# keiserlab/amyloid-yolo-paper

Hardware: AMD Instinct MI355X
Metric: tiles/sec (1024x1024 RGB) inference (higher is better)
Workload: dtype bf16; 1 GPU; configs[1]: Darknet-53+FPN YOLOv3, batch=64 synthetic 1024x1024 tiles/GPU, C=3, seeded random weights, decode + merge-NMS on (conf 0.5, nms 0.4); global_batch=64, tile=1024, parallelism=replicas x1 (tiles sharded by image, no collective)

## Files before the change

### amyloid_yolo_paper_amd/_lib.py

```python
import ctypes as C
import os

HERE = os.path.dirname(os.path.abspath(__file__))
LIB_PATH = os.path.join(HERE, "libamyloid_yolo_hip.so")
ABI_VERSION = 2


class ConvDesc(C.Structure):
    _fields_ = [(n, C.c_int32) for n in (
        "batch", "cin", "cout", "hin", "win", "hout", "wout", "ksize", "stride", "leaky", "out_f32", "cout_pad")]


class PlanOp(C.Structure):
    _fields_ = [("kind", C.c_int32), ("src", C.c_int32), ("src2", C.c_int32), ("res", C.c_int32), ("dst", C.c_int32),
                ("conv", ConvDesc), ("c1", C.c_int32), ("c2", C.c_int32), ("up1", C.c_int32), ("leaky2", C.c_int32),
                ("num_anchors", C.c_int32), ("num_classes", C.c_int32), ("grid", C.c_int32), ("row_offset", C.c_int32),
                ("anchors_wh", C.c_float * 12),
                ("w", C.c_void_p), ("scale", C.c_void_p), ("shift", C.c_void_p),
                ("w2", C.c_void_p), ("scale2", C.c_void_p), ("shift2", C.c_void_p)]


class AugParams(C.Structure):
    _fields_ = [("src_offset", C.c_int64), ("h", C.c_int32), ("w", C.c_int32), ("inv", C.c_float * 6), ("flip", C.c_int32),
                ("sharpen_alpha", C.c_float), ("drop_threshold", C.c_uint32), ("drop_seed", C.c_uint32),
# ... 43 lines not shown
    "ay_bn_train_bwd_f32": (_I, [_P, _P, _P, _P, _P, _P, _I, _P, _P, _P, _I, _I, _I, _P]),
    "ay_bias_grad_f32": (_I, [_P, _P, _I, _I, _I, _P]),
    "ay_bias_grad_f32_acc": (_I, [_P, _P, _I, _I, _I, _I, _P]),
    "ay_conv_dgrad_f32": (_I, [C.POINTER(ConvDesc), _P, _P, _P, _I, _P]),
    "ay_conv_wgrad_f32": (_I, [C.POINTER(ConvDesc), _P, _P, _P, _P]),
    "ay_add_f32": (_I, [_P, _P, _P, _SZ, _P]),
    "ay_accumulate_f32": (_I, [_P, _P, _SZ, _P]),
    "ay_copy_channels_f32": (_I, [_P, _P, _I, _I, _I, _I, _I, _I, _I, _P]),
    "ay_slice_accumulate_f32": (_I, [_P, _P, _I, _I, _I, _I, _I, _I, _I, _P]),
    "ay_yolo_loss_workspace_bytes": (_SZ, [_I, _I, _I, _I]),
    "ay_yolo_loss_fwd_bwd": (_I, [_P, _P, _I, _I, _I, _I, _I, _I, C.POINTER(C.c_float), _F, _F, _P, _P, _P, _SZ, _P]),
    "ay_conv1x1_cat_fwd_bf16": (_I, [C.POINTER(ConvDesc), _P, _I, _P, _P, _P, _P, _P, _P]),
    "ay_resblock_supported": (_I, [_I]),
    "ay_plan_create": (_I, [C.POINTER(PlanOp), _I, C.POINTER(C.c_size_t), _I, _I, _I, _I, C.POINTER(C.c_void_p)]),
    "ay_plan_destroy": (None, [_P]),
    "ay_plan_workspace_bytes": (_SZ, [_P]),
    "ay_plan_value_offset": (_SZ, [_P, _I]),
    "ay_plan_forward": (_I, [_P, _P, _P, _P, _P]),
    "ay_plan_forward_timed": (_I, [_P, _P, _P, _P, C.POINTER(C.c_float), _P]),
    "ay_plan_profile_begin": (_I, [_P, C.POINTER(C.c_ubyte)]),
    "ay_plan_profile_begin_every": (_I, [_P, C.POINTER(C.c_ubyte), _I]),
    "ay_plan_profile_end": (_I, [_P, C.POINTER(C.c_float), C.POINTER(C.c_int)]),
    "ay_resblock_fwd_bf16": (_I, [_P, _P, _P, _P, _I, _P, _P, _P, _I, _P, _I, _I, _I, _I, _P]),
    "ay_match_detections": (_I, [_P, _P, _I, _I, _P, _I, _F, _P, _P, _P]),
    "ay_ingest_tiles_u8": (_I, [_P, _I, _I, _I, _I, _F, _P, _P]),
    "ay_ingest_region_tiles_u8": (_I, [_P, _I, _I, _SZ, _I, _I, _I, _I, _I, _P, _P]),
    "ay_ingest_region_tiles_step_u8": (_I, [_P, _I, _I, _SZ, _I, _I, _I, _I, _I, _I, _P, _P]),
    "ay_ingest_region_tiles_list_u8": (_I, [_P, _I, _I, _SZ, _I, _I, _P, _I, _I, _P, _P]),
    "ay_augment_ingest_u8": (_I, [_P, _SZ, _P, _I, _I, _P, _P]),
    "ay_augment_ingest_window_u8": (_I, [_P, _SZ, _P, _I, _I, _P, _P]),
# ... 99 lines not shown
```

### amyloid_yolo_paper_amd/csrc/ay_conv3x3_m16.hip

```cpp
#include <type_traits>

#include "ay_conv_common.h"

namespace ay {

#ifdef AY_PHASE_CLOCK
__device__ unsigned long long g_phase_ticks_m16[10];
#define AY_CLK(...) __VA_ARGS__
#else
#define AY_CLK(...)
#endif

template <bool HAS_RES, typename DT = Bf16>
__global__ void __launch_bounds__(512, 2) conv3x3_m16_ring_kernel(ConvArgs a, int n_items) {
    DT::enter();
    typedef typename DT::vec8 vec8;
    constexpr int BN = 128, TH = 16, TW = 32;
    constexpr int IN_W = TW + 2, IN_PIX = (TH + 2) * IN_W;
    constexpr int IN_PIXP = (IN_PIX + 15) / 16 * 16;
    constexpr int PX_PIECES = (2 * IN_PIXP + 63) / 64;
    constexpr int PIX_SLAB = PX_PIECES * 1024;
    constexpr int W_PIECES = 9 * 2 * BN * 16 / 1024;
    constexpr int W_SLAB = W_PIECES * 1024;
    constexpr int W_BASE = PIX_SLAB;
// ... 5 lines not shown
    constexpr int SS_BASE = DUMMY_BASE + 1024;
    constexpr int MBOX_BASE = SS_BASE + 4 * 2048;
    constexpr int LDS_BYTES = MBOX_BASE + 64;
    static_assert(LDS_BYTES <= 160 * 1024, "LDS ring");
    constexpr int MT = 4, NT = 8;

    __shared__ __attribute__((aligned(16))) uint8_t lds[LDS_BYTES];
    __builtin_amdgcn_s_setprio(2);

    const int tid = threadIdx.x;
    const int lane = tid & 63;
    const int wave = __builtin_amdgcn_readfirstlane(tid >> 6);
    const int wm = wave & 1, wn = wave >> 1;
    const int r = lane & 15, g = lane >> 4, h = g & 1, hi = g >> 1;

    const ItemRange rg(n_items);
    const int last = rg.last;
    int item = rg.first_item();
    const ItemDealer dealer(rg, a.deal, lds + MBOX_BASE, 3);
    if (item >= last) {
        dealer.leave();
        return;
    }
    dealer.post_first();
    int seq_l = 0, seq_c = 0;

    const size_t in_plane = (size_t)a.hin * a.win * 32;
    const int CP = a.cout_pad;
    const size_t w_stage_stride = (size_t)9 * 2 * CP * 16;
    const int tiles_per_img = a.tiles_x * a.tiles_y;
    const unsigned lds_base = lds_addr_of(lds);
    const int nstages = a.cin / 16;

    constexpr unsigned OOB = 0x80000000u;
    unsigned px_off[PWP];
    const uint8_t* ld_src = nullptr;
    int ld_cg = 0;
    int ld_item = item, ld_s = 0, ld_par = 0;
    bool ld_done = false;
    auto setup_loader = [&](int it) __attribute__((always_inline)) {
        ld_cg = it % a.n_cgroups;
        const int pt = it / a.n_cgroups;
        const int b = pt / tiles_per_img;
        const int y0 = ((pt / a.tiles_x) % a.tiles_y) * TH, x0 = (pt % a.tiles_x) * TW;
        ld_src = a.src + (size_t)b * (a.cin / 16) * in_plane;
#pragma unroll
        for (int i = 0; i < PWP; ++i) {
            const int q = i * 8 + wave;
            const int u = q * 64 + lane;
            const int hh = u / IN_PIXP, P = u % IN_PIXP;
            const int iy = y0 - 1 + P / IN_W, ix = x0 - 1 + P % IN_W;
            const bool in = q < PX_PIECES && hh < 2 && P < IN_PIX && iy >= 0 && iy < a.hin && ix >= 0 && ix < a.win;
            px_off[i] = in ? (unsigned)((iy * a.win + ix) * 32 + hh * 16) : OOB;
        }
    };
// ... 39 lines not shown
    const int was = W_BASE + ((16 + h) * BN + wm * 64 + r) * 16 + hi * BUF_BYTES;

    setup_loader(item);
#pragma unroll
    for (int i = 0; i < PW; ++i) issue_piece(i, 0);
    advance_loader();
    asm volatile("s_waitcnt vmcnt(0)" ::: "memory");
    __builtin_amdgcn_s_barrier();
    asm volatile("" ::: "memory");

    int par = 0;
    AY_CLK(const bool clk = (a.dbg & 8) && wave == 0; unsigned long long tk_stage = 0, tk_epi = 0, tk_items = 0, tk_wait = 0, tk_wait0 = 0, tk_str = 0, tk0 = 0, tkw = 0;
           const unsigned long long tk_begin = wall_clock64();)
    while (true) {
        AY_CLK(if (clk) tk0 = wall_clock64();)
        const int cg = item % a.n_cgroups;
        const int pt = item / a.n_cgroups;
        const int b = pt / tiles_per_img;
        const int y0 = ((pt / a.tiles_x) % a.tiles_y) * TH, x0 = (pt % a.tiles_x) * TW;
        const int next_item = dealer.id_at(seq_c + 1);
        const bool has_next = next_item < last;

        f32x4 acc[MT][NT];
#pragma unroll
        for (int m = 0; m < MT; ++m)
#pragma unroll
            for (int n = 0; n < NT; ++n) acc[m][n] = f32x4{0.f, 0.f, 0.f, 0.f};

        typedef __attribute__((address_space(3))) const f32x4 lds_f4;
        lds_f4* sl4 = (lds_f4*)(__attribute__((address_space(3))) const float*)(lds + SS_BASE + par * 2048);
        const float slope = a.leaky ? 0.1f : 1.0f;
        const size_t out_plane_px = (size_t)a.hout * a.wout;
// ... 233 lines not shown
```

### amyloid_yolo_paper_amd/csrc/ay_conv_bf16.hip

```cpp
#include <stdlib.h>

#include <atomic>
#include <mutex>

#include "ay_conv_common.h"

namespace ay {

template <int KS, int STRIDE, int BN, int WM, int WN, int TH, int TW, int NK, bool OUT_F32, bool HAS_RES, typename DT = Bf16, bool DECODE = false>
__global__ void __launch_bounds__(256, 2) conv_bf16_kernel(ConvArgs a, DecodeArgs dd) {
    DT::enter();
    typedef typename DT::vec8 vec8;
    constexpr int PAD = (KS - 1) / 2;
    constexpr int KK2 = KS * KS;
    constexpr int NPIX = TH * TW;
    constexpr int NT = NPIX / (WN * 32);
    constexpr int MT = BN / (WM * 32);
    constexpr int IN_H = (TH - 1) * STRIDE + KS;
    constexpr int IN_W = (TW - 1) * STRIDE + KS;
    constexpr int IN_PIX = IN_H * IN_W;
    constexpr int PIX_SLAB = 2 * IN_PIX * 16;
    constexpr int W_SLAB = KK2 * 2 * BN * 16;
    constexpr int W_BASE = NK * PIX_SLAB;
    constexpr int LDS_BYTES = NK * (PIX_SLAB + W_SLAB);
// ... 1 lines not shown
    constexpr int NPXU = (PXU_TOTAL + 255) / 256;
    constexpr int WU_TOTAL = NK * KK2 * 2 * BN;
    constexpr int NWU = (WU_TOTAL + 255) / 256;
    static_assert(WM * WN == 4 && NT >= 1 && MT >= 1, "4 waves");
    static_assert(NT * WN * 32 == NPIX && MT * WM * 32 == BN, "tile split");
    static_assert(LDS_BYTES <= 80 * 1024, "two workgroups per CU");

    __shared__ __attribute__((aligned(16))) uint8_t lds[LDS_BYTES];

    const int tid = threadIdx.x;
    const int lane = tid & 63;
    const int wave = tid >> 6;
    const int wm = wave % WM, wn = wave / WM;
    const int c = lane & 31, hh = lane >> 5;

    const int bid = blockIdx.x;
    const int cg = bid % a.n_cgroups;
    const int pt = bid / a.n_cgroups;
    const int tile_x = pt % a.tiles_x;
    const int tile_y = (pt / a.tiles_x) % a.tiles_y;
    const int b = pt / (a.tiles_x * a.tiles_y);
    const int y0 = tile_y * TH, x0 = tile_x * TW;

    const size_t in_plane = (size_t)a.hin * a.win * 32;
    const uint8_t* src_img = a.src + (size_t)b * (a.cin / 16) * in_plane;
    const int CP = a.cout_pad;
    const uint8_t* wbase = a.w + (size_t)cg * BN * 16;
    const size_t w_stage_stride = (size_t)NK * KK2 * 2 * CP * 16;

    int px_off[NPXU];
#pragma unroll
// ... 155 lines not shown
    static_assert(WM * WN == 8 && NT >= 1 && MT >= 1, "8 waves");
    static_assert(NT * WN * 32 == NPIX && MT * WM * 32 == BN, "tile split");
    static_assert((KK2 * 2 * BN * 16) % 1024 == 0, "filter slab is whole DMA pieces");
    static_assert(LDS_BYTES <= 160 * 1024, "LDS ring");
    static_assert(NBUF == 2 || NBUF == 3, "ring depth");

    __shared__ __attribute__((aligned(16))) uint8_t lds[LDS_BYTES];
    __builtin_amdgcn_s_setprio(2);

    const int tid = threadIdx.x;
    const int lane = tid & 63;
    const int wave = __builtin_amdgcn_readfirstlane(tid >> 6);
    const int wm = wave % WM, wn = wave / WM;
    const int c = lane & 31, hh = lane >> 5;

    const ItemRange rg(n_items);
    const int last = rg.last;
    int item = rg.first_item();
    const ItemDealer dealer(rg, a.deal, lds + MBOX_BASE, (a.cin / (16 * NK)) >= 2 ? 3 : 5);
    if (item >= last) {
        dealer.leave();
        return;
    }
    dealer.post_first();
    int seq_l = 0, seq_c = 0;

    const size_t in_plane = (size_t)a.hin * a.win * 32;
    const int CP = a.cout_pad;
    const size_t w_stage_stride = (size_t)NK * KK2 * 2 * CP * 16;
    const int tiles_per_img = a.tiles_x * a.tiles_y;
    const unsigned lds_base = lds_addr_of(lds);
// ... 18 lines not shown
    for (int i = 0; i < PWW; ++i) {
        const int qq = i * 8 + wave;
        const int u = qq * 64 + lane;
        const int r = u % BN, th = u / BN;
        unsigned off = OOB;
        if (qq < NK * W_PIECES) {
            if constexpr (PAIR)
                off = (unsigned)((th * CP + r % (BN / 2)) * 16) + (unsigned)(r / (BN / 2)) * a.w_class_stride;
            else
                off = (unsigned)((th * CP + r) * 16);
        } else if (qq < NK * W_PIECES + SSP && lane < BN / 4) {
            off = (unsigned)(((lane * 4) % BNR) * 4);
        }
        w_off[i] = off;
    }
    auto setup_loader = [&](int it) __attribute__((always_inline)) {
        int cg = it % a.n_cgroups;
        const int pt = it / a.n_cgroups;
        const int b = pt / tiles_per_img;
        const int y0 = ((pt / a.tiles_x) % a.tiles_y) * TH, x0 = (pt % a.tiles_x) * TW;
        ld_src = a.src + (size_t)b * src_planes * in_plane;
        if constexpr (CAT) ld_src1 = a.src1 + (size_t)b * (a.c1 / 16) * in_plane1;
        const uint8_t* wbase = a.w;
        if constexpr (PAIR) {
            wbase += (size_t)((cg & 1) * 2) * a.w_class_stride;
            cg >>= 1;
        } else if constexpr (UP2) {
            wbase += (size_t)(cg & 3) * a.w_class_stride;
            cg >>= 2;
        }
        ld_w = wbase + (size_t)cg * BNR * 16;
// ... 96 lines not shown
            asm volatile("s_waitcnt vmcnt(0)" ::: "memory");
        }
    } else {
        asm volatile("s_waitcnt vmcnt(0)" ::: "memory");
    }
    __builtin_amdgcn_s_barrier();
    asm volatile("" ::: "memory");

    int cur = 0;
    int par = 0;
    const bool clk = AY_DBGBIT(a, 8) && wave == 0;
    unsigned long long tk_stage = 0, tk_epi = 0, tk_items = 0, tk0 = 0, tk_begin = 0, tk_s0 = 0, tk_w0 = 0, tk_w = 0, tk_nw = 0, tkw = 0;
    if (clk) tk_begin = wall_clock64();
    while (true) {
        if (clk) tk0 = wall_clock64();
        int cg = item % a.n_cgroups;
        const int cls = PAIR ? (cg & 1) * 2 : UP2 ? (cg & 3) : 0;
        if constexpr (PAIR)
            cg >>= 1;
        else if constexpr (UP2)
            cg >>= 2;
        const int pt = item / a.n_cgroups;
        const int b = pt / tiles_per_img;
        const int y0 = ((pt / a.tiles_x) % a.tiles_y) * TH, x0 = (pt % a.tiles_x) * TW;
        const int next_item = dealer.id_at(seq_c + 1);
        const bool has_next = next_item < last;

        f32x16 acc[MT][NT];
#pragma unroll
        for (int m = 0; m < MT; ++m)
#pragma unroll
            for (int n = 0; n < NT; ++n)
#pragma unroll
                for (int r = 0; r < 16; ++r) acc[m][n][r] = 0.f;
        ResRegs<MT, NT> rr;

        for (int s = 0; s < nstages; ++s) {
// ... 186 lines not shown
    a.cout_pad = d->cout_pad;
    a.hin = d->hin;
    a.win = d->win;
    a.hout = d->hout;
    a.wout = d->wout;
    a.tiles_x = (d->wout + TW - 1) / TW;
    a.tiles_y = (d->hout + TH - 1) / TH;
    a.n_cgroups = d->cout_pad / BN;
    a.leaky = d->leaky;
    a.dbg = 0;
    a.src1 = nullptr;
    a.c1 = 0;
    a.deal = nullptr;
    a.canvas_gx = 0;
    a.w_class_stride = 0;
}

int conv_dbg() {
    static const int dbg = getenv("AY_DBG") ? atoi(getenv("AY_DBG")) : 0;
    return dbg;
}

unsigned persistent_grid(long long n_items, int wgs_per_cu) {
    if (n_items <= 0 || n_items > 0x7fffffffLL) return 0;
    const long long per_xcd = (n_items + 7) / 8;
    const long long cu_slots = (long long)wgs_per_cu * (conv_num_cus() / 8);
    return (unsigned)(8 * (per_xcd < cu_slots ? per_xcd : cu_slots));
}

static long long plan_tiles(ConvArgs& a, const ay_conv_desc* d, int th, int tw, bool canvas_ok) {
    int ctx = 0, cty = 0;
// ... 251 lines not shown
```

### amyloid_yolo_paper_amd/csrc/ay_conv_common.h

```cpp
#pragma once
#include "ay_common.h"

#ifdef AY_PHASE_CLOCK
#define AY_DBGBIT(a, bit) ((a).dbg & (bit))
#else
#define AY_DBGBIT(a, bit) 0
#endif

namespace ay {

struct ConvArgs {
    const uint8_t* src;
    const uint8_t* w;
    const float* scale;
    const float* shift;
    const uint8_t* residual;
    uint8_t* out;
    int batch, cin, cout_pad, hin, win, hout, wout;
    int tiles_x, tiles_y, n_cgroups;
    int leaky;
    int dbg;
    const uint8_t* src1;
    int c1;
    unsigned* deal;
    int canvas_gx;
    unsigned w_class_stride;
};

struct DecodeArgs {
    float* pred;
    int n_total;
    int row_offset;
    int A, K;
    float stride;
    float aw[6], ah[6];
};

struct ItemRange {
    int xcd, slot, slots, first, last;
    __device__ __forceinline__ explicit ItemRange(int n_items) {
        xcd = blockIdx.x & 7, slot = blockIdx.x >> 3, slots = gridDim.x >> 3;
        const int per_xcd = (n_items + 7) >> 3;
        first = xcd * per_xcd;
        last = min(first + per_xcd, n_items);
    }
    __device__ __forceinline__ int first_item() const { return first + slot; }
};

struct ItemDealer {
    typedef volatile __attribute__((address_space(3))) int lds_vint;
    const ItemRange& rg;
    unsigned* deal;
    lds_vint* mbox;
    int D;
    __device__ __forceinline__ ItemDealer(const ItemRange& rg, unsigned* deal, void* mbox_lds, int D)
        : rg(rg), deal(deal), mbox((lds_vint*)(__attribute__((address_space(3))) int*)mbox_lds), D(D) {}
    __device__ __forceinline__ void leave() const {
        if (deal != nullptr && threadIdx.x == 0) {
            const unsigned d = atomicAdd(deal + 8, 1u);
            if (d == gridDim.x - 1) {
#pragma unroll
// ... 274 lines not shown
                } else {
#pragma unroll
                    for (int j = 0; j < 4; ++j) {
                        const int ch = ch0 + j;
                        const int an = ch / dd.K, k = ch - an * dd.K;
                        if (ch < dd.A * dd.K) rows[(size_t)an * G * G * dd.K + k] = res[j];
                    }
                }
            }
        }
    }
}

int conv_num_cus();
int conv_dbg();
unsigned* next_deal_set(hipStream_t st);
void fill_args(ConvArgs& a, const ay_conv_desc* d, const void* src, const void* w, const float* scale, const float* shift,
               const void* residual, void* out, int TH, int TW, int BN);
unsigned persistent_grid(long long n_items, int wgs_per_cu = 1);

inline int launch_ring(void (*kernel)(ConvArgs, int), ConvArgs a, long long n_items, bool dynamic, hipStream_t st, const char* what,
                       const char* kernel_name) {
    const unsigned grid = persistent_grid(n_items);
    if (!grid) {
        set_error("%s grid out of range (%lld)", what, n_items);
        return AY_ERR_ARG;
    }
    a.deal = dynamic ? next_deal_set(st) : nullptr;
    hipLaunchKernelGGL(kernel, dim3(grid), dim3(512), 0, st, a, (int)n_items);
    AY_CHECK_LAUNCH(kernel_name);
// ... 5 lines not shown
```

### amyloid_yolo_paper_amd/csrc/ay_plan.hip

```cpp
#include <hip/hip_runtime.h>

#include <algorithm>
#include <cstring>
#include <mutex>
#include <vector>

#include "ay_common.h"

struct ay_plan {
    std::vector<ay_plan_op> ops;
    std::vector<size_t> bytes, offset;
    std::vector<int> def_op, last_use;
    size_t arena = 0;
    int img_dim = 0, n_total = 0;
    int dtype = AY_DT_BF16;
    std::vector<int> fused;
    mutable bool profiling = false;
    mutable int prof_every = 1, prof_seen = 0;
    mutable std::vector<std::vector<hipEvent_t>> prof_events;
    std::vector<unsigned char> prof_sel;
};

namespace {

constexpr size_t ALIGN = 256;

bool uses_src2(int kind) { return kind == AY_OP_CONV1X1_CAT || kind == AY_OP_CONCAT_UPSAMPLE; }

void op_reads(const ay_plan_op& o, int (&r)[3]) {
    r[0] = (o.kind == AY_OP_STEM_S2_FUSED || o.kind == AY_OP_STEM) ? AY_PLAN_NONE : o.src;
    r[1] = uses_src2(o.kind) ? o.src2 : AY_PLAN_NONE;
// ... 1 lines not shown
}

struct Entries {
    decltype(&ay_head_decode_fwd_bf16) head_decode;
    decltype(&ay_stem_s2_fused_fwd) stem_s2_fused;
    decltype(&ay_stem_conv_fwd) stem;
    decltype(&ay_conv_fwd_bf16) conv;
    decltype(&ay_resblock_fwd_bf16) resblock;
    decltype(&ay_conv1x1_cat_fwd_bf16) conv1x1_cat;
};
constexpr Entries ENTRIES_BF16 = {ay_head_decode_fwd_bf16, ay_stem_s2_fused_fwd, ay_stem_conv_fwd,
                                  ay_conv_fwd_bf16,        ay_resblock_fwd_bf16, ay_conv1x1_cat_fwd_bf16};
constexpr Entries ENTRIES_F16 = {ay_head_decode_fwd_f16, ay_stem_s2_fused_fwd_f16, ay_stem_conv_fwd_f16,
                                 ay_conv_fwd_f16,        ay_resblock_fwd_f16,      ay_conv1x1_cat_fwd_f16};

int issue(const ay_plan* p, size_t idx, const float* x, uint8_t* ws, float* out, ay_stream_t st) {
    const ay_plan_op& o = p->ops[idx];
    const Entries& fn = p->dtype == AY_DT_F16 ? ENTRIES_F16 : ENTRIES_BF16;
    auto at = [&](int v) -> void* { return v >= 0 ? ws + p->offset[v] : nullptr; };
    const ay_conv_desc& d = o.conv;
    if (p->fused[idx] < 0) return AY_OK;
    if (p->fused[idx] > 0) {
        const ay_plan_op& y = p->ops[p->fused[idx]];
        return fn.head_decode(&d, at(o.src), o.w, o.scale, o.shift, y.num_anchors, y.num_classes, p->img_dim, y.anchors_wh, out,
                              p->n_total, y.row_offset, st);
    }
    switch (o.kind) {
        case AY_OP_STEM_S2_FUSED:
            return fn.stem_s2_fused(x, o.w, o.scale, o.shift, d.leaky, o.w2, o.scale2, o.shift2, o.leaky2, at(o.dst), d.batch, p->img_dim,
                                    p->img_dim, st);
        case AY_OP_STEM:
// ... 3 lines not shown
        case AY_OP_RESBLOCK:
            return fn.resblock(at(o.src), o.w, o.scale, o.shift, d.leaky, o.w2, o.scale2, o.shift2, o.leaky2, at(o.dst), d.batch, d.cin,
                               d.hout, d.wout, st);
        case AY_OP_CONV1X1_CAT:
            return fn.conv1x1_cat(&d, at(o.src), o.c1, at(o.src2), o.w, o.scale, o.shift, at(o.dst), st);
        case AY_OP_CONCAT_UPSAMPLE:
            return ay_concat_upsample_bf16(at(o.src), o.c1, o.up1, at(o.src2), o.c2, at(o.dst), d.batch, d.hout, d.wout, st);
        case AY_OP_DECODE:
            return ay_yolo_decode(static_cast<const float*>(at(o.src)), 1, out, d.batch, o.num_anchors, o.num_classes, o.grid,
                                  p->img_dim, o.anchors_wh, p->n_total, o.row_offset, st);
    }
    ay::set_error("ay_plan: unknown op kind %d", o.kind);
    return AY_ERR_ARG;
}

}

extern "C" int ay_plan_create(const ay_plan_op* ops, int n_ops, const size_t* value_bytes, int n_values, int img_dim,
                              int n_total_rows, int act_dtype, ay_plan** out_plan) {
    AY_CHECK_ARG(act_dtype == AY_DT_BF16 || act_dtype == AY_DT_F16, "ay_plan_create: activation dtype %d", act_dtype);
    AY_CHECK_ARG(ops && value_bytes && out_plan && n_ops > 0 && n_values > 0, "ay_plan_create: null / empty argument");
    AY_CHECK_ARG(img_dim > 0 && img_dim % 32 == 0 && n_total_rows > 0, "ay_plan_create: image side %d, %d rows", img_dim, n_total_rows);
    ay_plan* p = new ay_plan;
    p->ops.assign(ops, ops + n_ops);
    p->bytes.assign(value_bytes, value_bytes + n_values);
    p->offset.assign(n_values, 0);
    p->def_op.assign(n_values, -1);
    p->last_use.assign(n_values, -1);
    p->img_dim = img_dim;
    p->n_total = n_total_rows;
// ... 47 lines not shown
    std::sort(order.begin(), order.end(), [&](int a, int b) { return p->def_op[a] < p->def_op[b]; });
    for (int v : order) {
        const int born = p->def_op[v];
        live.erase(std::remove_if(live.begin(), live.end(), [&](const Live& l) { return l.until < born; }), live.end());
        std::sort(live.begin(), live.end(), [](const Live& a, const Live& b) { return a.off < b.off; });
        const size_t need = (p->bytes[v] + ALIGN - 1) / ALIGN * ALIGN;
        size_t off = 0;
        for (const Live& l : live) {
            if (off + need <= l.off) break;
            off = std::max(off, l.off + l.size);
        }
        p->offset[v] = off;
        live.push_back({off, need, p->last_use[v]});
        p->arena = std::max(p->arena, off + need);
    }
    *out_plan = p;
    return AY_OK;
}

extern "C" void ay_plan_destroy(ay_plan* plan) { delete plan; }

extern "C" size_t ay_plan_workspace_bytes(const ay_plan* plan) { return plan ? plan->arena : 0; }

extern "C" size_t ay_plan_value_offset(const ay_plan* plan, int value) {
    return (plan && value >= 0 && value < (int)plan->offset.size()) ? plan->offset[value] : (size_t)-1;
}

extern "C" int ay_plan_forward(const ay_plan* plan, const float* x_nchw, void* workspace, float* out_rows, ay_stream_t stream) {
    AY_CHECK_ARG(plan && x_nchw && workspace && out_rows, "ay_plan_forward: null argument");
    std::vector<hipEvent_t>* ev = nullptr;
    hipStream_t st = ay::S(stream);
    if (plan->profiling && (plan->prof_seen++ % plan->prof_every) == 0) {
// ... 108 lines not shown
```

### amyloid_yolo_paper_amd/csrc/ay_resblock_bf16.hip

```cpp
#include "ay_conv_common.h"

namespace ay {

__device__ __attribute__((aligned(64))) uint32_t g_zero_page_rb[16];

struct ResBlockArgs {
    const uint8_t* x;
    const uint8_t* w1;
    const uint8_t* w2;
    const float* scale1;
    const float* shift1;
    int leaky1;
    ConvArgs c2;
};

template <int CM, int TH, int NKA, int NBUF, typename DT = Bf16>
__global__ void __launch_bounds__(512, 2) resblock_bf16_kernel(ResBlockArgs s, int n_items) {
    DT::enter();
    typedef typename DT::vec8 vec8;
    constexpr int C = 2 * CM;
    constexpr int TW = 32, IN_W = TW + 2, IN_H = TH + 2;
    constexpr int HP = IN_H * IN_W;
    constexpr int NPB = (HP + 31) / 32;
    constexpr int HPP = NPB * 32;
// ... 19 lines not shown
    constexpr int WMA = CM / 32, WNA = 8 / WMA, NBA = (NPB + WNA - 1) / WNA;
    constexpr int WM = BN2 / 64, WN = 8 / WM, MT = 2, NT = (TH * TW) / (WN * 32);
    static_assert(MT * WM * 32 == BN2 && NT * WN * 32 == TH * TW, "tile split");
    static_assert(MT * NT <= 4, "32 VGPRs of residual held from phase A to the epilogue");

    __shared__ __attribute__((aligned(16))) uint8_t lds[LDS_BYTES];
    __builtin_amdgcn_s_setprio(2);
    const ConvArgs& a = s.c2;
    const int tid = threadIdx.x;
    const int lane = tid & 63;
    const int wave = __builtin_amdgcn_readfirstlane(tid >> 6);
    const int c = lane & 31, hh = lane >> 5;
    const int wma = wave % WMA, wna = wave / WMA;
    const int wm = wave % WM, wn = wave / WM;

    const ItemRange rg(n_items);
    const int slots = rg.slots, last = rg.last;
    int item = rg.first_item();
    if (item >= last) return;

    const int H = a.hout, W = a.wout;
    const size_t plane_bytes = (size_t)H * W * 32;
    const int tiles_per_img = a.tiles_x * a.tiles_y;
    const uint8_t* zero_page = reinterpret_cast<const uint8_t*>(g_zero_page_rb);
    const unsigned lds_base = lds_addr_of(lds);

    {
        float* ss1 = reinterpret_cast<float*>(lds + OFF_SS1);
        float* ss2 = reinterpret_cast<float*>(lds + OFF_SS2);
        if (tid < CM) {
            ss1[tid] = s.scale1[tid];
            ss1[CM + tid] = s.shift1[tid];
        }
        if (tid < BN2) {
            ss2[tid] = a.scale[tid];
            ss2[128 + tid] = a.shift[tid];
        }
    }

    int xoff[PW];
    const uint8_t* ld_xbase = nullptr;
    int ld_item = item, ld_ls = 0;
    bool ld_done = false;
    auto setup_loader = [&](int it) __attribute__((always_inline)) {
        const int b = it / tiles_per_img;
        const int y0 = ((it / a.tiles_x) % a.tiles_y) * TH, x0 = (it % a.tiles_x) * TW;
        ld_xbase = s.x + (size_t)b * (C / 16) * plane_bytes;
#pragma unroll
        for (int i = 0; i < PW; ++i) {
            const int q = i * 8 + wave;
            int off = -1;
            if (q < A_PIECES) {
                const int r = q % (XP + W1P);
                if (r < XP) {
                    const int u = r * 64 + lane;
                    const int h = u / HP, P = u % HP;
                    const int iy = y0 - 1 + P / IN_W, ix = x0 - 1 + P % IN_W;
                    if (h < 2 && iy >= 0 && iy < H && ix >= 0 && ix < W) off = (iy * W + ix) * 32 + h * 16;
                }
// ... 62 lines not shown
        const int p = (wn * NT + n) * 32 + c;
        rp[n] = (hh * HP + (p / TW + 1) * IN_W + (p % TW + 1)) * 16;
    }
    const int wa2 = (hh * BN2 + wm * MT * 32 + c) * 16;
    const int wa1 = XP * 1024 + (hh * CM + wma * 32 + c) * 16;

    static_assert(SA + SB >= NBUF - 1, "an item has at least NBUF-1 stages");
    setup_loader(item);
#pragma unroll
    for (int k = 0; k < NBUF - 1; ++k) issue_stage(k);
    asm volatile("s_waitcnt vmcnt(%0)" ::"n"((NBUF - 2) * PW) : "memory");
    __syncthreads();

    int cur = 0;
    while (true) {
        const int b = item / tiles_per_img;
        const int y0 = ((item / a.tiles_x) % a.tiles_y) * TH, x0 = (item % a.tiles_x) * TW;
        const int next_item = item + slots;
        const bool has_next = next_item < last;

        ResRegs<MT, NT> rr;
        f32x16 accA[NBA];
#pragma unroll
        for (int j = 0; j < NBA; ++j)
#pragma unroll
            for (int r = 0; r < 16; ++r) accA[j][r] = 0.f;
        for (int sa = 0; sa < SA; ++sa) {
            const bool issued = !ld_done;
            int slot_ld = cur + (NBUF - 1);
            if (slot_ld >= NBUF) slot_ld -= NBUF;
            const uint8_t* L = lds + cur * SLOT;
#pragma unroll
// ... 170 lines not shown
```

### amyloid_yolo_paper_amd/csrc/ay_stem_fused.hip

```cpp
#include "ay_conv_common.h"

namespace ay {

__device__ __attribute__((aligned(64))) uint32_t g_zero_page_st[16];
#ifdef AY_PHASE_CLOCK
__device__ unsigned long long g_stem_ticks[8];
#define STEM_TICK(k)                                   \
    if (wave == 0) {                                   \
        const unsigned long long t_ = wall_clock64();  \
        tk[k] += t_ - tk_last;                         \
        tk_last = t_;                                  \
    }
#else
#define STEM_TICK(k)
#endif

struct StemFusedArgs {
    const float* x;
    const uint16_t* w0;
    const float* scale0;
    const float* shift0;
    int leaky0;
    int H, W;
    unsigned m_tx, m_tpi;
// ... 22 lines not shown
    constexpr int OFF_SS0 = OFF_W1 + W1_BYTES;
    constexpr int OFF_SS1 = OFF_SS0 + 256;
    constexpr int LDS_BYTES = OFF_SS1 + 1024;
    static_assert(LDS_BYTES <= 160 * 1024, "LDS");
    constexpr int MT = 1, NT = 1;

    __shared__ __attribute__((aligned(16))) uint8_t lds[LDS_BYTES];
    __builtin_amdgcn_s_setprio(2);

    const int tid = threadIdx.x;
    const int lane = tid & 63;
    const int wave = __builtin_amdgcn_readfirstlane(tid >> 6);
    const int c = lane & 31, hh = lane >> 5;
    const ConvArgs& a = s.c1;

    const ItemRange rg(n_items);
    const int slots = rg.slots, last = rg.last;
    int item = rg.first_item();
    if (item >= last) return;
    const int tiles_per_img = a.tiles_x * a.tiles_y;

    for (int u = tid; u < W1_BYTES / 16; u += NT_)
        *reinterpret_cast<uint4*>(lds + OFF_W1 + u * 16) = *reinterpret_cast<const uint4*>(reinterpret_cast<const uint8_t*>(a.w) + (size_t)u * 16);
    vec8 wa[2];
#pragma unroll
    for (int ks = 0; ks < 2; ++ks) wa[ks] = *reinterpret_cast<const vec8*>(s.w0 + c * 32 + 16 * ks + 8 * hh);
    asm volatile("" ::"v"(wa[0]), "v"(wa[1]));

    auto koff = [](int k) constexpr { return k < 27 ? ((k / 9) * IH + (k % 9) / 3) * IW + k % 3 : -1; };
    float* ss0 = reinterpret_cast<float*>(lds + OFF_SS0);
    if (tid < 32) {
        ss0[tid] = s.scale0[tid];
        ss0[32 + tid] = s.shift0[tid];
    }
    if (tid < BN) {
        float* ss1 = reinterpret_cast<float*>(lds + OFF_SS1);
        ss1[tid] = a.scale[tid];
        ss1[128 + tid] = a.shift[tid];
    }

    const uint8_t* zero_page = reinterpret_cast<const uint8_t*>(g_zero_page_st);
    const unsigned lds_base = lds_addr_of(lds);
    auto issue_image = [&](int it, int slot_i) __attribute__((always_inline)) {
        const int b = it / tiles_per_img;
        const int y0 = ((it / a.tiles_x) % a.tiles_y) * TH, x0 = (it % a.tiles_x) * TW;
        const float* xb = s.x + (size_t)b * 3 * s.H * s.W;
#pragma unroll 1
        for (int i = 0; i < NDMA; ++i) {
            const int k = i * 16 + wave;
            const void* g = zero_page + (lane & 15) * 4;
            int dst = NIB * IMG_BYTES;
            if (k < IMG_DMAS) {
                const int u = k * 64 + lane;
                if (u < IMG_ELEMS) {
                    const int col = u % IW, r = (u / IW) % IH, ci = u / (IW * IH);
                    const int iy = 2 * y0 - 2 + r, ix = 2 * x0 - 2 + col;
                    if (iy >= 0 && iy < s.H && ix >= 0 && ix < s.W) g = xb + ((size_t)ci * s.H + iy) * s.W + ix;
                }
// ... 11 lines not shown
    {
        const int it1 = item + slots;
        if (it1 < last) {
            issue_image(it1, 1);
            asm volatile("s_waitcnt vmcnt(%0)" ::"n"(NDMA) : "memory");
        } else {
            asm volatile("s_waitcnt vmcnt(0)" ::: "memory");
        }
    }
    __syncthreads();
    int ib = 0;
#ifdef AY_PHASE_CLOCK
    unsigned long long tk[8] = {0, 0, 0, 0, 0, 0, 0, 0}, tk_last = wall_clock64();
#endif
    while (true) {
        const int pt = item;
        const int b = pt / tiles_per_img;
        const int y0 = ((pt / a.tiles_x) % a.tiles_y) * TH, x0 = (pt % a.tiles_x) * TW;
        const int next_item = item + slots;
        const bool has_next = next_item < last;
        const bool has_next2 = next_item + slots < last;
        const float* img = reinterpret_cast<const float*>(lds + ib * IMG_BYTES);
        if (has_next2) issue_image(next_item + slots, ib >= 1 ? ib - 1 : NIB - 1);
        STEM_TICK(0)

        for (int blk = wave; blk < S_PIXP / 32; blk += 16) {
            const int P = blk * 32 + c;
            const int sy = P / SW, sx = P % SW;
            const bool inside = P < S_PIX;
            const int ibase = inside ? sy * IW + sx : 0;
            f32x16 acc;
// ... 118 lines not shown
    constexpr int LDS_BYTES = OFF_SS1 + 1024;
    static_assert(LDS_BYTES <= 160 * 1024, "LDS");
    static_assert(IMG_DMAS <= 16, "one tile DMA per wave");
    constexpr int MT = 1, NT = 1;
    constexpr unsigned OOB = 0x80000000u;

    __shared__ __attribute__((aligned(16))) uint8_t lds[LDS_BYTES];
    __builtin_amdgcn_s_setprio(2);

    const int tid = threadIdx.x;
    const int lane = tid & 63;
    const int wave = __builtin_amdgcn_readfirstlane(tid >> 6);
    const int c = lane & 31, hh = lane >> 5;
    const ConvArgs& a = s.c1;

    const ItemRange rg(n_items);
    if (rg.first_item() >= rg.last) return;
    const int nk = (rg.last - rg.first_item() + rg.slots - 1) / rg.slots;
    const unsigned tiles_per_img = (unsigned)(a.tiles_x * a.tiles_y);
    struct Coord { int b, y0, x0; };
    auto coord_of = [&](int k) __attribute__((always_inline)) {
        const unsigned it = (unsigned)(rg.first_item() + k * rg.slots);
        unsigned b = __umulhi(it, s.m_tpi), r = it - b * tiles_per_img;
        if (r >= tiles_per_img) ++b, r -= tiles_per_img;
        unsigned ty = __umulhi(r, s.m_tx), tx = r - ty * (unsigned)a.tiles_x;
        if (tx >= (unsigned)a.tiles_x) ++ty, tx -= (unsigned)a.tiles_x;
        return Coord{(int)b, (int)ty * TH, (int)tx * TW};
    };

    if (tid < BN) {
        float* ss1 = reinterpret_cast<float*>(lds + OFF_SS1);
        ss1[tid] = a.scale[tid];
        ss1[128 + tid] = a.shift[tid];
    }
    const unsigned lds_base = lds_addr_of(lds);
    const int pu = wave * 64 + lane;
    const bool pu_ok = wave < IMG_DMAS && pu < IMG_PIECES;
// ... 276 lines not shown
```

### amyloid_yolo_paper_amd/models.py

```python
import ctypes as C
import os
from typing import NamedTuple

import numpy as np
import torch
import torch.nn as nn

from . import _lib
from ._lib import ConvDesc, check, ptr
from .parse_config import parse_model_config


class Upsample(nn.Module):

    def __init__(self, scale_factor, mode="nearest"):
        super().__init__()
        self.scale_factor, self.mode = scale_factor, mode


class EmptyLayer(nn.Module):
    """route / shortcut placeholder."""


class YOLOLayer(nn.Module):
# ... 86 lines not shown
        self.img_size = img_size
        self.seen = 0
        self.header_info = np.array([0, 0, 0, self.seen, 0], dtype=np.int32)
        assert precision in ("bf16", "fp16", "fp32")
        self.precision = precision
        self.fuse_block_channels = (64,)
        self._graph = self._analyse()
        self._prep = None
        self._act_bufs = {}
        self.keep_layer_outputs = False
        self.layer_outputs = None
        self.stem_mode = "fused_bf16"
        self.fold_routes = True
        self.fuse_blocks = True
        self.use_plan = os.environ.get("AY_USE_PLAN", "1") != "0"
        self.box_loss = "mse"

    def _analyse(self):
        defs = self.module_defs
        n = len(defs)
        ch = []
        info = []
        cin = int(self.hyperparams["channels"])
        scale = []
        for i, d in enumerate(defs):
            t = d["type"]
            e = {"type": t}
            prev_ch = ch[-1] if ch else cin
            prev_sc = scale[-1] if scale else 0
            if t == "convolutional":
# ... 439 lines not shown
    def _lower_key(self, B, S):
        return (B, S, self.precision, self.fuse_blocks, self.fold_routes, self.stem_mode, tuple(self.fuse_block_channels),
                self.keep_layer_outputs)

    def _lowered(self, B, S, prep):
        cache = prep.setdefault("lowered", {})
        key = self._lower_key(B, S)
        if key not in cache:
            cache[key] = self._lower(B, S, prep)
        for y, e in zip(self.yolo_layers, (g for g in self._graph if g["type"] == "yolo")):
            y.grid_size, y.img_dim = S >> e["log2_down"], S
        return cache[key]

    def _plan(self, B, S, prep, dev):
        plans = prep.setdefault("plans", {})
        key = self._lower_key(B, S)
        if key not in plans:
            assert self._mfma
            L = _lib.lib()
            low = self._lowered(B, S, prep)
            arr = (_lib.PlanOp * len(low.ops))(*low.ops)
            vb = (C.c_size_t * len(low.value_bytes))(*low.value_bytes)
            handle = C.c_void_p()
            check(L.ay_plan_create(arr, len(low.ops), vb, len(vb), S, self.num_boxes(S), int(self.precision == "fp16"), C.byref(handle)),
                  "ay_plan_create")
            ws = torch.empty(L.ay_plan_workspace_bytes(handle), device=dev, dtype=torch.uint8)
            plans[key] = _Plan(handle, ws, low)
        return plans[key]

    def plan_profile_begin(self, B, S, layers=None, every=1):
        dev = torch.device("cuda", torch.cuda.current_device())
        plan = self._plan(B, S, self._prepare(dev), dev)
        sel = None
        if layers is not None:
            sel = (C.c_ubyte * len(plan.ops))(*[int(layer in layers) for layer in plan.op_layer])
        check(_lib.lib().ay_plan_profile_begin_every(plan.handle, sel, int(every)), "ay_plan_profile_begin")

    def plan_profile_end(self, B, S):
        dev = torch.device("cuda", torch.cuda.current_device())
        plan = self._plan(B, S, self._prepare(dev), dev)
# ... 28 lines not shown
```

### include/amyloid_yolo.h

```cpp
#ifndef AMYLOID_YOLO_H
#define AMYLOID_YOLO_H

#include <stddef.h>
#include <stdint.h>

#ifdef __cplusplus
extern "C" {
#endif

#define AY_OK 0
#define AY_ERR_ARG (-1)
#define AY_ERR_LAUNCH (-2)
#define AY_ERR_WORKSPACE (-3)

typedef void* ay_stream_t;

#define AY_DT_BF16 0
#define AY_DT_F16 1

#define AY_ABI_VERSION 2
int ay_version(void);
const char* ay_last_error(void);

typedef struct ay_conv_desc {
// ... 9 lines not shown


int ay_pack_conv_weights_bf16(const float* w_oihw, void* packed, int cout, int cout_pad, int cin, int ksize,
                              ay_stream_t stream);
size_t ay_packed_weight_bytes(int cout_pad, int cin, int ksize);

int ay_fold_bn(const float* gamma, const float* beta, const float* mean, const float* var, const float* bias,
               float eps, float* scale, float* shift, int n, int n_pad, ay_stream_t stream);

int ay_stem_conv_fwd(const float* x_nchw, const float* w_oihw, const float* scale, const float* shift,
                     void* out_blocked, int batch, int h, int w, int leaky, ay_stream_t stream);

int ay_stem_s2_fused_fwd(const float* x_nchw, const void* stem_w_bf16, const float* scale0, const float* shift0, int leaky0,
                         const void* w1_packed, const float* scale1, const float* shift1, int leaky1, void* out_blocked,
                         int batch, int h, int w, ay_stream_t stream);

int ay_conv_fwd_bf16(const ay_conv_desc* d, const void* src, const void* w_packed, const float* scale,
                     const float* shift, const void* residual, void* out, ay_stream_t stream);

int ay_conv3x3_m16_fwd_bf16(const ay_conv_desc* d, const void* src, const void* w_packed, const float* scale, const float* shift,
                            const void* residual, void* out, ay_stream_t stream);

int ay_conv1x1_cat_fwd_bf16(const ay_conv_desc* d, const void* src1_halfres, int c1, const void* src2, const void* w_packed,
                            const float* scale, const float* shift, void* out, ay_stream_t stream);

int ay_resblock_supported(int channels);
int ay_resblock_fwd_bf16(const void* x, const void* w1_packed, const float* scale1, const float* shift1, int leaky1,
                         const void* w2_packed, const float* scale2, const float* shift2, int leaky2, void* out, int batch,
                         int channels, int h, int w, ay_stream_t stream);

// ... 213 lines not shown
    int32_t num_anchors, num_classes, grid, row_offset;
    float anchors_wh[12];
    const void* w;
    const float* scale;
    const float* shift;
    const void* w2;
    const float* scale2;
    const float* shift2;
} ay_plan_op;
typedef struct ay_plan ay_plan;
int ay_plan_create(const ay_plan_op* ops, int n_ops, const size_t* value_bytes, int n_values, int img_dim, int n_total_rows,
                   int act_dtype, ay_plan** out_plan);
void ay_plan_destroy(ay_plan* plan);
size_t ay_plan_workspace_bytes(const ay_plan* plan);
size_t ay_plan_value_offset(const ay_plan* plan, int value);
int ay_plan_forward(const ay_plan* plan, const float* x_nchw, void* workspace, float* out_rows, ay_stream_t stream);
int ay_plan_profile_begin(ay_plan* plan, const unsigned char* op_selected);
int ay_plan_profile_begin_every(ay_plan* plan, const unsigned char* op_selected, int every);
int ay_plan_profile_end(ay_plan* plan, float* op_ms_sum , int* n_forwards);
int ay_plan_forward_timed(const ay_plan* plan, const float* x_nchw, void* workspace, float* out_rows, float* op_ms,
                          ay_stream_t stream);

int ay_merge_detections_max_rows(void);
int ay_merge_detections(const float* rows, const int* count, int batch, int max_rows, float* rows_out, int* count_out,
                        ay_stream_t stream);

#define AY_SEAM_FLAG_MAX_DET 1
#define AY_SEAM_FLAG_CAPACITY 2
int ay_seam_append(const float* rows, const int32_t* count, int batch, int max_det, float scale, const float* origins_xy,
                   const int32_t* tile_ids, float* slide_rows, int32_t* slide_tile, int32_t* slide_count, int capacity,
// ... 41 lines not shown
```

Baseline: 2688 tiles/s.

## Alternate tile traversal direction across plan ops for cache reuse

Adds a reverse traversal mode to the persistent conv, resblock and stem kernels, so each XCD walks its item range backwards. The plan picks a direction per op so a consumer reads its largest input in the order opposite to how the producer wrote it. The aim is that the most recently written tiles, still resident in L2/MALL, are consumed first. It adds a thread-local traversal flag and an index remap in every kernel, and it can disturb existing locality patterns such as weight reuse across cgroups.

Result: faster. 2733 tiles/s, median of 6 (+1.7%).

```diff
diff --git a/amyloid_yolo_paper_amd/_lib.py b/amyloid_yolo_paper_amd/_lib.py
--- a/amyloid_yolo_paper_amd/_lib.py
+++ b/amyloid_yolo_paper_amd/_lib.py
@@ -81,6 +81,10 @@
     "ay_resblock_supported": (_I, [_I]),
     "ay_plan_create": (_I, [C.POINTER(PlanOp), _I, C.POINTER(C.c_size_t), _I, _I, _I, _I, C.POINTER(C.c_void_p)]),
     "ay_plan_destroy": (None, [_P]),
+    "ay_plan_set_alternation": (_I, [_P, _I]),
+    "ay_plan_op_reversed": (_I, [_P, _I]),
+    "ay_conv_set_traversal": (None, [_I]),
+    "ay_conv_get_traversal": (_I, []),
     "ay_plan_workspace_bytes": (_SZ, [_P]),
     "ay_plan_value_offset": (_SZ, [_P, _I]),
     "ay_plan_forward": (_I, [_P, _P, _P, _P, _P]),
diff --git a/amyloid_yolo_paper_amd/csrc/ay_conv3x3_m16.hip b/amyloid_yolo_paper_amd/csrc/ay_conv3x3_m16.hip
--- a/amyloid_yolo_paper_amd/csrc/ay_conv3x3_m16.hip
+++ b/amyloid_yolo_paper_amd/csrc/ay_conv3x3_m16.hip
@@ -43,7 +43,7 @@
     const int wm = wave & 1, wn = wave >> 1;
     const int r = lane & 15, g = lane >> 4, h = g & 1, hi = g >> 1;
 
-    const ItemRange rg(n_items);
+    const ItemRange rg(n_items, a.reverse);
     const int last = rg.last;
     int item = rg.first_item();
     const ItemDealer dealer(rg, a.deal, lds + MBOX_BASE, 3);
@@ -67,7 +67,8 @@
     int ld_cg = 0;
     int ld_item = item, ld_s = 0, ld_par = 0;
     bool ld_done = false;
-    auto setup_loader = [&](int it) __attribute__((always_inline)) {
+    auto setup_loader = [&](int id) __attribute__((always_inline)) {
+        const int it = rg.item_of(id);
         ld_cg = it % a.n_cgroups;
         const int pt = it / a.n_cgroups;
         const int b = pt / tiles_per_img;
@@ -137,8 +138,9 @@
            const unsigned long long tk_begin = wall_clock64();)
     while (true) {
         AY_CLK(if (clk) tk0 = wall_clock64();)
-        const int cg = item % a.n_cgroups;
-        const int pt = item / a.n_cgroups;
+        const int it = rg.item_of(item);
+        const int cg = it % a.n_cgroups;
+        const int pt = it / a.n_cgroups;
         const int b = pt / tiles_per_img;
         const int y0 = ((pt / a.tiles_x) % a.tiles_y) * TH, x0 = (pt % a.tiles_x) * TW;
         const int next_item = dealer.id_at(seq_c + 1);
diff --git a/amyloid_yolo_paper_amd/csrc/ay_conv_bf16.hip b/amyloid_yolo_paper_amd/csrc/ay_conv_bf16.hip
--- a/amyloid_yolo_paper_amd/csrc/ay_conv_bf16.hip
+++ b/amyloid_yolo_paper_amd/csrc/ay_conv_bf16.hip
@@ -39,7 +39,7 @@
     const int wm = wave % WM, wn = wave / WM;
     const int c = lane & 31, hh = lane >> 5;
 
-    const int bid = blockIdx.x;
+    const int bid = a.reverse ? gridDim.x - 1 - blockIdx.x : blockIdx.x;
     const int cg = bid % a.n_cgroups;
     const int pt = bid / a.n_cgroups;
     const int tile_x = pt % a.tiles_x;
@@ -225,7 +225,7 @@
     const int wm = wave % WM, wn = wave / WM;
     const int c = lane & 31, hh = lane >> 5;
 
-    const ItemRange rg(n_items);
+    const ItemRange rg(n_items, a.reverse);
     const int last = rg.last;
     int item = rg.first_item();
     const ItemDealer dealer(rg, a.deal, lds + MBOX_BASE, (a.cin / (16 * NK)) >= 2 ? 3 : 5);
@@ -274,7 +274,8 @@
         }
         w_off[i] = off;
     }
-    auto setup_loader = [&](int it) __attribute__((always_inline)) {
+    auto setup_loader = [&](int id) __attribute__((always_inline)) {
+        const int it = rg.item_of(id);
         int cg = it % a.n_cgroups;
         const int pt = it / a.n_cgroups;
         const int b = pt / tiles_per_img;
@@ -401,13 +402,14 @@
     if (clk) tk_begin = wall_clock64();
     while (true) {
         if (clk) tk0 = wall_clock64();
-        int cg = item % a.n_cgroups;
+        const int it = rg.item_of(item);
+        int cg = it % a.n_cgroups;
         const int cls = PAIR ? (cg & 1) * 2 : UP2 ? (cg & 3) : 0;
         if constexpr (PAIR)
             cg >>= 1;
         else if constexpr (UP2)
             cg >>= 2;
-        const int pt = item / a.n_cgroups;
+        const int pt = it / a.n_cgroups;
         const int b = pt / tiles_per_img;
         const int y0 = ((pt / a.tiles_x) % a.tiles_y) * TH, x0 = (pt % a.tiles_x) * TW;
         const int next_item = dealer.id_at(seq_c + 1);
@@ -624,7 +626,15 @@
     a.deal = nullptr;
     a.canvas_gx = 0;
     a.w_class_stride = 0;
-}
+    a.reverse = conv_traversal_reverse();
+}
+
+static thread_local int t_traversal_reverse = 0;
+int conv_traversal_reverse() { return t_traversal_reverse; }
+}
+extern "C" void ay_conv_set_traversal(int reverse) { ay::t_traversal_reverse = reverse != 0; }
+extern "C" int ay_conv_get_traversal(void) { return ay::t_traversal_reverse; }
+namespace ay {
 
 int conv_dbg() {
     static const int dbg = getenv("AY_DBG") ? atoi(getenv("AY_DBG")) : 0;
diff --git a/amyloid_yolo_paper_amd/csrc/ay_conv_common.h b/amyloid_yolo_paper_amd/csrc/ay_conv_common.h
--- a/amyloid_yolo_paper_amd/csrc/ay_conv_common.h
+++ b/amyloid_yolo_paper_amd/csrc/ay_conv_common.h
@@ -25,6 +25,7 @@
     unsigned* deal;
     int canvas_gx;
     unsigned w_class_stride;
+    int reverse;
 };
 
 struct DecodeArgs {
@@ -38,13 +39,16 @@
 
 struct ItemRange {
     int xcd, slot, slots, first, last;
-    __device__ __forceinline__ explicit ItemRange(int n_items) {
+    int flip;
+    __device__ __forceinline__ explicit ItemRange(int n_items, int reverse = 0) {
         xcd = blockIdx.x & 7, slot = blockIdx.x >> 3, slots = gridDim.x >> 3;
         const int per_xcd = (n_items + 7) >> 3;
         first = xcd * per_xcd;
         last = min(first + per_xcd, n_items);
+        flip = reverse ? first + last - 1 : -1;
     }
     __device__ __forceinline__ int first_item() const { return first + slot; }
+    __device__ __forceinline__ int item_of(int id) const { return flip >= 0 ? flip - id : id; }
 };
 
 struct ItemDealer {
@@ -349,6 +353,7 @@
 
 int conv_num_cus();
 int conv_dbg();
+int conv_traversal_reverse();
 unsigned* next_deal_set(hipStream_t st);
 void fill_args(ConvArgs& a, const ay_conv_desc* d, const void* src, const void* w, const float* scale, const float* shift,
                const void* residual, void* out, int TH, int TW, int BN);
diff --git a/amyloid_yolo_paper_amd/csrc/ay_plan.hip b/amyloid_yolo_paper_amd/csrc/ay_plan.hip
--- a/amyloid_yolo_paper_amd/csrc/ay_plan.hip
+++ b/amyloid_yolo_paper_amd/csrc/ay_plan.hip
@@ -15,6 +15,8 @@
     int img_dim = 0, n_total = 0;
     int dtype = AY_DT_BF16;
     std::vector<int> fused;
+    std::vector<unsigned char> reverse;
+    bool alternate = false;
     mutable bool profiling = false;
     mutable int prof_every = 1, prof_seen = 0;
     mutable std::vector<std::vector<hipEvent_t>> prof_events;
@@ -46,7 +48,7 @@
 constexpr Entries ENTRIES_F16 = {ay_head_decode_fwd_f16, ay_stem_s2_fused_fwd_f16, ay_stem_conv_fwd_f16,
                                  ay_conv_fwd_f16,        ay_resblock_fwd_f16,      ay_conv1x1_cat_fwd_f16};
 
-int issue(const ay_plan* p, size_t idx, const float* x, uint8_t* ws, float* out, ay_stream_t st) {
+int issue_op(const ay_plan* p, size_t idx, const float* x, uint8_t* ws, float* out, ay_stream_t st) {
     const ay_plan_op& o = p->ops[idx];
     const Entries& fn = p->dtype == AY_DT_F16 ? ENTRIES_F16 : ENTRIES_BF16;
     auto at = [&](int v) -> void* { return v >= 0 ? ws + p->offset[v] : nullptr; };
@@ -80,6 +82,33 @@
     return AY_ERR_ARG;
 }
 
+int issue(const ay_plan* p, size_t idx, const float* x, uint8_t* ws, float* out, ay_stream_t st) {
+    if (!p->alternate) return issue_op(p, idx, x, ws, out, st);
+    const int before = ay_conv_get_traversal();
+    ay_conv_set_traversal(p->reverse[idx]);
+    const int rc = issue_op(p, idx, x, ws, out, st);
+    ay_conv_set_traversal(before);
+    return rc;
+}
+
+void choose_directions(ay_plan* p) {
+    const size_t n = p->ops.size();
+    p->reverse.assign(n, 0);
+    std::vector<unsigned char> touched_rev(p->bytes.size(), 0);
+    for (size_t i = 0; i < n; ++i) {
+        const ay_plan_op& o = p->ops[i];
+        const bool persistent = o.kind == AY_OP_STEM_S2_FUSED || o.kind == AY_OP_CONV || o.kind == AY_OP_RESBLOCK || o.kind == AY_OP_CONV1X1_CAT;
+        int r[3];
+        op_reads(o, r);
+        int big = AY_PLAN_NONE;
+        for (int v : r)
+            if (v >= 0 && (big < 0 || p->bytes[v] > p->bytes[big])) big = v;
+        p->reverse[i] = persistent && big >= 0 && !touched_rev[big];
+        for (int v : r)
+            if (v >= 0) touched_rev[v] = p->reverse[i];
+        if (o.kind != AY_OP_DECODE) touched_rev[o.dst] = p->reverse[i];
+    }
+}
 }
 
 extern "C" int ay_plan_create(const ay_plan_op* ops, int n_ops, const size_t* value_bytes, int n_values, int img_dim,
@@ -157,8 +186,19 @@
         live.push_back({off, need, p->last_use[v]});
         p->arena = std::max(p->arena, off + need);
     }
+    choose_directions(p);
     *out_plan = p;
     return AY_OK;
+}
+
+extern "C" int ay_plan_set_alternation(ay_plan* plan, int on) {
+    AY_CHECK_ARG(plan, "ay_plan_set_alternation: null plan");
+    plan->alternate = on != 0;
+    return AY_OK;
+}
+
+extern "C" int ay_plan_op_reversed(const ay_plan* plan, int op) {
+    return (plan && plan->alternate && op >= 0 && op < (int)plan->reverse.size()) ? plan->reverse[op] : 0;
 }
 
 extern "C" void ay_plan_destroy(ay_plan* plan) { delete plan; }
diff --git a/amyloid_yolo_paper_amd/csrc/ay_resblock_bf16.hip b/amyloid_yolo_paper_amd/csrc/ay_resblock_bf16.hip
--- a/amyloid_yolo_paper_amd/csrc/ay_resblock_bf16.hip
+++ b/amyloid_yolo_paper_amd/csrc/ay_resblock_bf16.hip
@@ -57,7 +57,7 @@
     const int wma = wave % WMA, wna = wave / WMA;
     const int wm = wave % WM, wn = wave / WM;
 
-    const ItemRange rg(n_items);
+    const ItemRange rg(n_items, a.reverse);
     const int slots = rg.slots, last = rg.last;
     int item = rg.first_item();
     if (item >= last) return;
@@ -85,7 +85,8 @@
     const uint8_t* ld_xbase = nullptr;
     int ld_item = item, ld_ls = 0;
     bool ld_done = false;
-    auto setup_loader = [&](int it) __attribute__((always_inline)) {
+    auto setup_loader = [&](int id) __attribute__((always_inline)) {
+        const int it = rg.item_of(id);
         const int b = it / tiles_per_img;
         const int y0 = ((it / a.tiles_x) % a.tiles_y) * TH, x0 = (it % a.tiles_x) * TW;
         ld_xbase = s.x + (size_t)b * (C / 16) * plane_bytes;
@@ -178,8 +179,9 @@
 
     int cur = 0;
     while (true) {
-        const int b = item / tiles_per_img;
-        const int y0 = ((item / a.tiles_x) % a.tiles_y) * TH, x0 = (item % a.tiles_x) * TW;
+        const int it = rg.item_of(item);
+        const int b = it / tiles_per_img;
+        const int y0 = ((it / a.tiles_x) % a.tiles_y) * TH, x0 = (it % a.tiles_x) * TW;
         const int next_item = item + slots;
         const bool has_next = next_item < last;
 
diff --git a/amyloid_yolo_paper_amd/csrc/ay_stem_fused.hip b/amyloid_yolo_paper_amd/csrc/ay_stem_fused.hip
--- a/amyloid_yolo_paper_amd/csrc/ay_stem_fused.hip
+++ b/amyloid_yolo_paper_amd/csrc/ay_stem_fused.hip
@@ -60,7 +60,7 @@
     const int c = lane & 31, hh = lane >> 5;
     const ConvArgs& a = s.c1;
 
-    const ItemRange rg(n_items);
+    const ItemRange rg(n_items, a.reverse);
     const int slots = rg.slots, last = rg.last;
     int item = rg.first_item();
     if (item >= last) return;
@@ -87,7 +87,8 @@
 
     const uint8_t* zero_page = reinterpret_cast<const uint8_t*>(g_zero_page_st);
     const unsigned lds_base = lds_addr_of(lds);
-    auto issue_image = [&](int it, int slot_i) __attribute__((always_inline)) {
+    auto issue_image = [&](int id, int slot_i) __attribute__((always_inline)) {
+        const int it = rg.item_of(id);
         const int b = it / tiles_per_img;
         const int y0 = ((it / a.tiles_x) % a.tiles_y) * TH, x0 = (it % a.tiles_x) * TW;
         const float* xb = s.x + (size_t)b * 3 * s.H * s.W;
@@ -129,7 +130,7 @@
     unsigned long long tk[8] = {0, 0, 0, 0, 0, 0, 0, 0}, tk_last = wall_clock64();
 #endif
     while (true) {
-        const int pt = item;
+        const int pt = rg.item_of(item);
         const int b = pt / tiles_per_img;
         const int y0 = ((pt / a.tiles_x) % a.tiles_y) * TH, x0 = (pt % a.tiles_x) * TW;
         const int next_item = item + slots;
@@ -278,13 +279,13 @@
     const int c = lane & 31, hh = lane >> 5;
     const ConvArgs& a = s.c1;
 
-    const ItemRange rg(n_items);
+    const ItemRange rg(n_items, a.reverse);
     if (rg.first_item() >= rg.last) return;
     const int nk = (rg.last - rg.first_item() + rg.slots - 1) / rg.slots;
     const unsigned tiles_per_img = (unsigned)(a.tiles_x * a.tiles_y);
     struct Coord { int b, y0, x0; };
     auto coord_of = [&](int k) __attribute__((always_inline)) {
-        const unsigned it = (unsigned)(rg.first_item() + k * rg.slots);
+        const unsigned it = (unsigned)rg.item_of(rg.first_item() + k * rg.slots);
         unsigned b = __umulhi(it, s.m_tpi), r = it - b * tiles_per_img;
         if (r >= tiles_per_img) ++b, r -= tiles_per_img;
         unsigned ty = __umulhi(r, s.m_tx), tx = r - ty * (unsigned)a.tiles_x;
diff --git a/amyloid_yolo_paper_amd/models.py b/amyloid_yolo_paper_amd/models.py
--- a/amyloid_yolo_paper_amd/models.py
+++ b/amyloid_yolo_paper_amd/models.py
@@ -124,6 +124,7 @@
         self.fold_routes = True
         self.fuse_blocks = True
         self.use_plan = os.environ.get("AY_USE_PLAN", "1") != "0"
+        self.alternate_traversal = os.environ.get("AY_PLAN_ALTERNATE", "1") != "0"
         self.box_loss = "mse"
 
     def _analyse(self):
@@ -593,7 +594,7 @@
 
     def _plan(self, B, S, prep, dev):
         plans = prep.setdefault("plans", {})
-        key = self._lower_key(B, S)
+        key = self._lower_key(B, S) + (bool(self.alternate_traversal),)
         if key not in plans:
             assert self._mfma
             L = _lib.lib()
@@ -603,6 +604,7 @@
             handle = C.c_void_p()
             check(L.ay_plan_create(arr, len(low.ops), vb, len(vb), S, self.num_boxes(S), int(self.precision == "fp16"), C.byref(handle)),
                   "ay_plan_create")
+            check(L.ay_plan_set_alternation(handle, int(bool(self.alternate_traversal))), "ay_plan_set_alternation")
             ws = torch.empty(L.ay_plan_workspace_bytes(handle), device=dev, dtype=torch.uint8)
             plans[key] = _Plan(handle, ws, low)
         return plans[key]
diff --git a/include/amyloid_yolo.h b/include/amyloid_yolo.h
--- a/include/amyloid_yolo.h
+++ b/include/amyloid_yolo.h
@@ -47,6 +47,9 @@
 int ay_stem_s2_fused_fwd(const float* x_nchw, const void* stem_w_bf16, const float* scale0, const float* shift0, int leaky0,
                          const void* w1_packed, const float* scale1, const float* shift1, int leaky1, void* out_blocked,
                          int batch, int h, int w, ay_stream_t stream);
+
+void ay_conv_set_traversal(int reverse);
+int ay_conv_get_traversal(void);
 
 int ay_conv_fwd_bf16(const ay_conv_desc* d, const void* src, const void* w_packed, const float* scale,
                      const float* shift, const void* residual, void* out, ay_stream_t stream);
@@ -290,6 +293,8 @@
 void ay_plan_destroy(ay_plan* plan);
 size_t ay_plan_workspace_bytes(const ay_plan* plan);
 size_t ay_plan_value_offset(const ay_plan* plan, int value);
+int ay_plan_set_alternation(ay_plan* plan, int on);
+int ay_plan_op_reversed(const ay_plan* plan, int op);
 int ay_plan_forward(const ay_plan* plan, const float* x_nchw, void* workspace, float* out_rows, ay_stream_t stream);
 int ay_plan_profile_begin(ay_plan* plan, const unsigned char* op_selected);
 int ay_plan_profile_begin_every(ay_plan* plan, const unsigned char* op_selected, int every);
```
